# jacobkrantz/IVLN-CE

Measured on AMD Instinct MI355X. Metric: env-steps/sec (batched MapCMA fwd+bwd) at 1/2/4/8 MI355X; t-nDTW parity, higher is better.
Workload: dtype f32

## Files before the change

### include/ivln_hip.h

```cpp
#ifndef IVLN_HIP_H
#define IVLN_HIP_H
#include <stdint.h>
#ifdef __cplusplus
extern "C" {
#endif

#define IVLN_OK 0
#define IVLN_E_INVALID -1
#define IVLN_E_HIP -2
#define IVLN_E_KEYSPACE -3
#define IVLN_E_CAPACITY -4
#define IVLN_E_UNSUPPORTED -5

const char* ivln_strerror(int code);
int ivln_version(void);

typedef struct ivln_mapper ivln_mapper;

int ivln_mapper_create(int B_max, int H, int W, double vfov_rad, double height_m, double width_m,
                       double res_m, int64_t world_capacity, int64_t table_cells, ivln_mapper** out);
int ivln_mapper_destroy(ivln_mapper* m);
int ivln_mapper_reset(ivln_mapper* m, void* stream);

int ivln_mapper_set_launch_width(ivln_mapper* m, int local_blocks, int world_blocks);
// ... 65 lines not shown
    int64_t ws_floats;
    int defer_epilogue;
    int* splits_used;
    int tile_override;
    const float* A_packed;
    int no_xcd_remap;
    int grp_imgs;
    int64_t a_grp_stride, a_packed_grp_stride;
    int no_wide_epilogue;
    float* stat_partials;
    int* stat_tiles;
    const void* A_split;
    int64_t a_split_grp_stride;
    int split_ok;
    const int32_t* img_run_flags;
    const void* fuse_A_split;
    int64_t fuse_a_grp_stride;
    const float* fuse_scale;
    const float* fuse_shift;
    int fuse_M;
    int residual_after_relu;
    int real_taps;
    int pool2;
    const uint8_t* map_sem_u8;
} ivln_gemm_desc;

int ivln_gemm_f32(const ivln_gemm_desc* desc, void* stream);
int64_t ivln_conv_split_words(int M, int Cin, int KS);
int ivln_conv_split_weights_f32(const float* W, int M, int Cin, int KS, void* out, void* stream);
int64_t ivln_conv_stem_split_words(int M, int Cin);
int ivln_conv_stem_split_weights_f32(const float* W, int M, int Cin, void* out, void* stream);
int ivln_conv_split_counters(double* flops, long long* launches, int reset);
int ivln_conv_split_kinds(long long* out4, int reset);

int ivln_family_timing_begin(int max_launches);
int ivln_family_timing_end(double* total_ms, int* launches, int* dropped);
int ivln_family_timing_report(char* buf, int cap);
const char* ivln_family_kernel_names(void);
int64_t ivln_conv_packed_floats(int M, int Cin, int KS);
int ivln_conv_pack_weights_f32(const float* W, int M, int Cin, int KS, float* out, void* stream);

typedef struct ivln_gn_conv_desc {
    const float* x;
    int splits;
    int64_t slab_stride;
    const float* gamma;
    const float* beta;
    const float* x2;
    int splits2;
    int64_t slab_stride2;
    const float* gamma2;
    const float* beta2;
    const float* residual;
    int N, C, H, W, groups;
    float eps;
    int relu;
    int pool;
    float* act_out;
    const float* wa;
    int Cout_a, ka, stride_a, pad_a;
    float* ya;
    const float* wb;
    int Cout_b, stride_b;
    float* yb;
    const float* x0;
    int splits0;
// ... 292 lines not shown
```

### ivln-ce_amd/csrc/conv_bf3.hip

```cpp
#include <stdlib.h>

#include <type_traits>

#include "gemm_common.h"
#include "residency.h"

namespace {

typedef __bf16 bf16x8 __attribute__((ext_vector_type(8)));
typedef int v4i __attribute__((ext_vector_type(4)));
typedef int v2i __attribute__((ext_vector_type(2)));

constexpr int PIXB = 112;
constexpr int CB = 16;

__host__ __device__ constexpr int bf3_taps_padded(int KS) { return KS == 7 ? 54 : (KS == 3 ? 9 : (KS == 2 ? 4 : 1)); }
__host__ __device__ constexpr int bf3_gx0(int KS) { return KS == 2 ? 0 : 4; }
__host__ __device__ constexpr int bf3_xoff(int KS) { return KS == 2 ? 0 : 4 - KS / 2; }
__host__ __device__ constexpr int bf3_stage_chunks(int KS) { return KS == 1 ? 4 : 1; }

__device__ __forceinline__ uint32_t bf16_rne_bits(float v, bool& fin) {
    const uint32_t u = __float_as_uint(v);
    fin = (u & 0x7F800000u) != 0x7F800000u;
    uint32_t hb = (u + 0x7FFFu + ((u >> 16) & 1u)) & 0xFFFF0000u;
// ... 1067 lines not shown
    if (!attr_done) {
        if (hipFuncSetAttribute((const void*)kern, hipFuncAttributeMaxDynamicSharedMemorySize, (int)lds) != hipSuccess) return IVLN_E_HIP;
        attr_done = true;
    }
    const int tiles_w = d.Wout / 8, tiles_h = d.Hout / 4;
    dim3 grid(tiles_w * tiles_h * nimg, (d.M + 31) / 32, 1);
    IVLN_LAUNCH_FAMILY_NAMED("k_conv7_pool_bf3", kern, grid, dim3(64 * NW), lds, s, d, (const unsigned char*)d.A_split, tiles_w, tiles_h, nimg);
    return IVLN_OK;
}

int bf3_conv7_pool_launch(ivln_gemm_desc& d, hipStream_t s) {
    if (d.bmode != BMODE_CONV_K7 || d.amode != AMODE_MK || d.dmode != DMODE_NCHW || d.dil != 1 || d.stride != 1 || d.pad != 3 ||
        d.Hout != d.Hin || d.Wout != d.Win || d.K != d.Cin * 49 || d.HoWo != d.Hout * d.Wout || d.N % d.HoWo != 0)
        return IVLN_E_UNSUPPORTED;
    if ((d.Hout & 3) || (d.Wout & 7) || !d.scale || !d.shift || !d.relu || d.residual || d.accumulate || d.residual_after_relu || d.defer_epilogue ||
        d.splits > 1 || d.stat_partials || d.img_run_flags || d.fuse_A_split || d.grp_imgs > 0 || d.Cin > 8 * CB)
        return IVLN_E_UNSUPPORTED;
    const int nimg = d.N / d.HoWo;
    const int64_t tiles = (int64_t)nimg * (d.Hout / 4) * (d.Wout / 8);
    if (tiles >= (int64_t)1 << 30) return IVLN_E_UNSUPPORTED;
    d.splits = 1;
    if (d.map_sem_u8) {
        if (d.Cin != 14 || (int64_t)nimg * d.HoWo >= (int64_t)1 << 31) return IVLN_E_UNSUPPORTED;
        return launch_conv7_pool<1, true>(d, s, nimg);
    }
    if ((d.in_img_stride & 3) || (((uintptr_t)d.B) & 15) || (int64_t)nimg * d.in_img_stride * 4 >= (int64_t)1 << 31) return IVLN_E_UNSUPPORTED;
    const int nch = (d.Cin + CB - 1) / CB;
    if (nch == 1) return launch_conv7_pool<1, false>(d, s, nimg);
    if (nch == 2) return launch_conv7_pool<2, false>(d, s, nimg);
    if (nch <= 4) return launch_conv7_pool<4, false>(d, s, nimg);
    return launch_conv7_pool<8, false>(d, s, nimg);
}

template <bool WT>
__global__ __launch_bounds__(WT ? 256 : 512, 2) void k_conv1x1_bf3_ks(const ivln_gemm_desc p, const unsigned char* a_split, long long a_grp_bytes) {
    constexpr int NW = WT ? 4 : 8, TN = 4, DA = 4, BN = 128;
    constexpr int LDT = BN + 4;
    constexpr unsigned OOB = 0x80000000u;
    extern __shared__ __attribute__((aligned(16))) unsigned char smem[];
    const int t = threadIdx.x, lane = t & 63;
    const int wave = __builtin_amdgcn_readfirstlane(t >> 6);
    const int half = lane >> 5, l31 = lane & 31;
    const BlockId bid = xcd_block_id(p.no_xcd_remap);
    const int n0 = WT ? (bid.y * NW + wave) * BN : bid.y * BN, m0 = bid.x * 32;
    const int nch = p.Cin / CB;
    const int HW = p.HoWo;
    const int cpw = WT ? nch : (nch + NW - 1) / NW;
    const int c0 = WT ? 0 : min(nch, wave * cpw), c1 = WT ? nch : min(nch, c0 + cpw);
    const int n_img0 = min(n0, p.N - 1) / HW;
    const int grp = p.grp_imgs > 0 ? n_img0 / p.grp_imgs : 0;

    const int nq = n0 + 4 * l31;
    const int qimg = nq / HW, qpp = nq - qimg * HW;
    const unsigned hw4 = (unsigned)HW * 4u;
    const unsigned xvo = nq < p.N ? (unsigned)(((int64_t)qimg * p.in_img_stride + qpp + (int64_t)(8 * half) * HW) * 4) : OOB;
    const __amdgpu_buffer_rsrc_t rB = bf3_rsrc(p.B);
    auto load_x = [&](int c, v4i (&xb)[8]) {
        const int so = c * CB * HW * 4;
#pragma unroll
        for (int j = 0; j < 8; ++j) xb[j] = __builtin_amdgcn_raw_buffer_load_b128(rB, (int)xvo, so + j * (int)hw4, 0);
    };
    const int mt = min(m0 / 32, (p.M + 31) / 32 - 1);
    const __amdgpu_buffer_rsrc_t rA = bf3_rsrc(a_split + (int64_t)grp * a_grp_bytes + (int64_t)mt * nch * (3 * 1024));
    const int c_last = max(c1 - 1, 0);
    auto load_a = [&](int c, v4i (&ab)[3]) {
#pragma unroll
        for (int pl = 0; pl < 3; ++pl) ab[pl] = __builtin_amdgcn_raw_buffer_load_b128(rA, (min(c, c_last) * 3 + pl) * 1024 + lane * 16, 0, 0);
    };
    f32x16 acc[TN];
#pragma unroll
    for (int tn = 0; tn < TN; ++tn)
#pragma unroll
        for (int i = 0; i < 16; ++i) acc[tn][i] = 0.f;

#ifdef BF3_TIMING
    const unsigned long long ts0 = lane == 0 ? wall_clock64() : 0ull;
    unsigned long long ts1 = ts0, tc_split = 0, tc_load = 0, tc_mfma = 0;
#endif
    if (c0 < c1 && (!WT || n0 < p.N)) {
        v4i xb[2][8], ab[DA][3];
#pragma unroll
        for (int d = 0; d < DA; ++d) load_a(c0 + d, ab[d]);
        load_x(c0, xb[0]);
        load_x(min(c0 + 1, c_last), xb[1]);
#ifdef BF3_TIMING
        __builtin_amdgcn_s_waitcnt(0);
        ts1 = lane == 0 ? wall_clock64() : 0ull;
#endif
        for (int cc = c0; cc < c1; cc += DA) {
#pragma unroll
            for (int k = 0; k < DA; ++k) {
                const int c = cc + k;
                v4i bq[TN][3];
                bf16x8 a[3];
#ifdef BF3_TIMING
                const unsigned long long tl0 = __builtin_readcyclecounter();
#endif
                if (c < c1) {
#pragma unroll
                    for (int e = 0; e < 4; ++e)
#pragma unroll
                        for (int i = 0; i < 4; ++i) {
                            uint32_t H, M, L;
#ifdef BF3_PROBE_NO_SPLIT
                            H = xb[k & 1][2 * i][e], M = xb[k & 1][2 * i + 1][e], L = H ^ M;
#else
                            split3_pair(__int_as_float(xb[k & 1][2 * i][e]), __int_as_float(xb[k & 1][2 * i + 1][e]), H, M, L);
#endif
                            bq[e][0][i] = (int)H, bq[e][1][i] = (int)M, bq[e][2][i] = (int)L;
                        }
#pragma unroll
                    for (int pl = 0; pl < 3; ++pl) a[pl] = __builtin_bit_cast(bf16x8, ab[k][pl]);
                }
                __builtin_amdgcn_sched_barrier(0);
#ifdef BF3_TIMING
                const unsigned long long tl1 = __builtin_readcyclecounter();
                __builtin_amdgcn_sched_barrier(0);
#endif
                load_x(min(c + 2, c_last), xb[k & 1]);
                load_a(c + DA, ab[k]);
                __builtin_amdgcn_sched_barrier(0);
#ifdef BF3_TIMING
                const unsigned long long tl2 = __builtin_readcyclecounter();
                __builtin_amdgcn_sched_barrier(0);
#endif
                if (c < c1) {
#define IVLN_BF3_PROD(PA, PB)                            \
    _Pragma("unroll") for (int tn = 0; tn < TN; ++tn)    \
        acc[tn] = __builtin_amdgcn_mfma_f32_32x32x16_bf16(a[PA], __builtin_bit_cast(bf16x8, bq[tn][PB]), acc[tn], 0, 0, 0)
#ifdef BF3_PROBE_NO_MFMA
                    IVLN_BF3_PROD(0, 0);
#else
                    IVLN_BF3_PROD(0, 2);
                    IVLN_BF3_PROD(1, 1);
                    IVLN_BF3_PROD(2, 0);
                    IVLN_BF3_PROD(0, 1);
                    IVLN_BF3_PROD(1, 0);
                    IVLN_BF3_PROD(0, 0);
#endif
#undef IVLN_BF3_PROD
                }
#ifdef BF3_TIMING
                __builtin_amdgcn_sched_barrier(0);
                const unsigned long long tl3 = __builtin_readcyclecounter();
                tc_split += tl1 - tl0, tc_load += tl2 - tl1, tc_mfma += tl3 - tl2;
#endif
            }
        }
    }
#ifdef BF3_TIMING
    const unsigned long long ts2 = lane == 0 ? wall_clock64() : 0ull;
#endif
    const bool up = p.dmode == DMODE_NCHW_UP2X4;
    if (WT && up) {
        const int n = n0 + 4 * l31;
        if (n < p.N) {
            const int img = n / HW, pp = n - img * HW;
            const int ho = pp / p.Wout, wo = pp - ho * p.Wout;
#pragma unroll
            for (int r = 0; r < 16; r += 2) {
                const int m = m0 + 4 * half + (r & 3) + 8 * (r >> 2);
                if (m >= p.M) continue;
                const int co = m >> 2, a = (m >> 1) & 1;
                const int64_t addr = (((int64_t)img * p.Ctot + co) * (2 * p.Hout) + 2 * ho + a) * (2 * p.Wout) + 2 * wo;
                float v[8];
#pragma unroll
                for (int e = 0; e < 4; ++e) v[2 * e] = acc[e][r], v[2 * e + 1] = acc[e][r + 1];
                const float sc = p.scale ? p.scale[co] : 1.f, sh = p.shift ? p.shift[co] : 0.f;
#pragma unroll
                for (int e = 0; e < 8; ++e) v[e] = p.scale ? fmaf(v[e], sc, sh) : v[e] + sh;
                if (p.residual) {
                    const float4 r0 = *reinterpret_cast<const float4*>(p.residual + addr), r1 = *reinterpret_cast<const float4*>(p.residual + addr + 4);
                    v[0] += r0.x, v[1] += r0.y, v[2] += r0.z, v[3] += r0.w, v[4] += r1.x, v[5] += r1.y, v[6] += r1.z, v[7] += r1.w;
                }
                if (p.relu) {
#pragma unroll
                    for (int e = 0; e < 8; ++e) v[e] = fmaxf(v[e], 0.f);
                }
                *reinterpret_cast<float4*>(p.D + addr) = make_float4(v[0], v[1], v[2], v[3]);
                *reinterpret_cast<float4*>(p.D + addr + 4) = make_float4(v[4], v[5], v[6], v[7]);
            }
        }
    } else
    if constexpr (WT) {
        const int n = n0 + 4 * l31;
        const int img = min(n, p.N - 1) / HW, pp = n - img * HW;
        const int mrem = n < p.N ? p.M - m0 - 4 * half : 0;
        const int me0 = (p.grp_imgs > 0 ? (img / p.grp_imgs) * p.M : 0) + m0 + 4 * half;
        const unsigned off0 = (unsigned)(((img * p.Ctot + m0 + 4 * half) * HW + pp) * 4);
        const __amdgpu_buffer_rsrc_t rR = bf3_rsrc(p.residual), rS = bf3_rsrc(p.scale), rH = bf3_rsrc(p.shift), rD = bf3_rsrc(p.D);
        const bool has_res = p.residual != nullptr, has_sc = p.scale != nullptr, has_sh = p.shift != nullptr;
        const float relu_lo = p.relu ? 0.f : -__builtin_huge_valf();
        const bool res_post = p.residual_after_relu != 0;
        v4i rres[16];
        float esc[16], esh[16];
#pragma unroll
        for (int r = 0; r < 16; ++r) {
            const int cs = (r & 3) + 8 * (r >> 2);
            const bool ok = cs < mrem;
            esc[r] = __int_as_float(__builtin_amdgcn_raw_buffer_load_b32(rS, ok && has_sc ? me0 * 4 : (int)OOB, cs * 4, 0));
            esh[r] = __int_as_float(__builtin_amdgcn_raw_buffer_load_b32(rH, ok && has_sh ? me0 * 4 : (int)OOB, cs * 4, 0));
            rres[r] = __builtin_amdgcn_raw_buffer_load_b128(rR, ok && has_res ? (int)off0 : (int)OOB, cs * HW * 4, 0);
        }
#pragma unroll
        for (int r = 0; r < 16; ++r) {
            const int cs = (r & 3) + 8 * (r >> 2);
            float4 v = make_float4(acc[0][r], acc[1][r], acc[2][r], acc[3][r]);
            const float sc = has_sc ? esc[r] : 1.f, sh = esh[r];
            v.x = fmaf(v.x, sc, sh), v.y = fmaf(v.y, sc, sh), v.z = fmaf(v.z, sc, sh), v.w = fmaf(v.w, sc, sh);
            const float r0 = __int_as_float(rres[r][0]), r1 = __int_as_float(rres[r][1]), r2 = __int_as_float(rres[r][2]), r3 = __int_as_float(rres[r][3]);
            v.x += res_post ? 0.f : r0, v.y += res_post ? 0.f : r1, v.z += res_post ? 0.f : r2, v.w += res_post ? 0.f : r3;
            const float lo = relu_lo;
            v.x = fmaxf(v.x, lo), v.y = fmaxf(v.y, lo), v.z = fmaxf(v.z, lo), v.w = fmaxf(v.w, lo);
            v.x += res_post ? r0 : 0.f, v.y += res_post ? r1 : 0.f, v.z += res_post ? r2 : 0.f, v.w += res_post ? r3 : 0.f;
            v4i o;
            o[0] = __float_as_int(v.x), o[1] = __float_as_int(v.y), o[2] = __float_as_int(v.z), o[3] = __float_as_int(v.w);
            __builtin_amdgcn_raw_buffer_store_b128(o, rD, cs < mrem ? (int)off0 : (int)OOB, cs * HW * 4, 0);
            BF3_STORE_GUARD();
        }
    } else if (up) {
        float* const red = reinterpret_cast<float*>(smem);
#pragma unroll
        for (int tn = 0; tn < TN; ++tn)
#pragma unroll
            for (int r = 0; r < 16; ++r)
                red[(wave * 32 + (r & 3) + 8 * (r >> 2) + 4 * half) * LDT + tn * 32 + l31] = acc[tn][r];
        __syncthreads();
#pragma unroll
        for (int it = 0; it < 2; ++it) {
            const int item = t + it * 512, r = item >> 6, j = item & 63;
            const int ml = 2 * r, nl = 2 * j, n = n0 + nl;
            const int e0 = nl & 3, q = nl >> 2;
            float4 v = make_float4(0.f, 0.f, 0.f, 0.f);
#pragma unroll
            for (int w = 0; w < NW; ++w) {
                const float* r0 = red + (w * 32 + ml) * LDT + q;
                const float* r1 = r0 + LDT;
                v.x += r0[e0 * 32], v.y += r1[e0 * 32], v.z += r0[(e0 + 1) * 32], v.w += r1[(e0 + 1) * 32];
            }
            if (m0 + ml < p.M && n < p.N) {
                const int img = n / HW, pp = n - img * HW;
                const int ho = pp / p.Wout, wo = pp - ho * p.Wout;
                const int co = (m0 + ml) >> 2, a = r & 1;
                const int64_t addr = (((int64_t)img * p.Ctot + co) * (2 * p.Hout) + 2 * ho + a) * (2 * p.Wout) + 2 * wo;
                if (p.scale) {
                    const float sc = p.scale[co], sh = p.shift[co];
                    v.x = fmaf(v.x, sc, sh), v.y = fmaf(v.y, sc, sh), v.z = fmaf(v.z, sc, sh), v.w = fmaf(v.w, sc, sh);
                } else if (p.shift) {
                    const float sh = p.shift[co];
                    v.x += sh, v.y += sh, v.z += sh, v.w += sh;
                }
                if (p.residual) {
                    const float4 rr = *reinterpret_cast<const float4*>(p.residual + addr);
                    v.x += rr.x, v.y += rr.y, v.z += rr.z, v.w += rr.w;
                }
                if (p.relu) v.x = fmaxf(v.x, 0.f), v.y = fmaxf(v.y, 0.f), v.z = fmaxf(v.z, 0.f), v.w = fmaxf(v.w, 0.f);
                *reinterpret_cast<float4*>(p.D + addr) = v;
            }
        }
    } else {
    constexpr int ITEMS = 2;
    v4i rres[ITEMS];
    float esc[ITEMS], esh[ITEMS];
    int eoff[ITEMS];
    const __amdgpu_buffer_rsrc_t rR = bf3_rsrc(p.residual), rS = bf3_rsrc(p.scale), rH = bf3_rsrc(p.shift);
    const bool has_res = p.residual != nullptr, has_sc = p.scale != nullptr, has_sh = p.shift != nullptr;
    auto request = [&](int it) {
        const int item = t + it * 512, ml = item >> 5, q = item & 31;
        const int m = m0 + ml, n = n0 + 4 * q;
        const bool ok = m < p.M && n < p.N;
        const int img = n / HW, pp = n - img * HW;
        const int off = (img * p.Ctot + m) * HW + pp;
        const int me = p.grp_imgs > 0 ? (img / p.grp_imgs) * p.M + m : m;
        eoff[it] = ok ? off : -1;
        esc[it] = __int_as_float(__builtin_amdgcn_raw_buffer_load_b32(rS, ok && has_sc ? me * 4 : (int)OOB, 0, 0));
        esh[it] = __int_as_float(__builtin_amdgcn_raw_buffer_load_b32(rH, ok && has_sh ? me * 4 : (int)OOB, 0, 0));
        rres[it] = __builtin_amdgcn_raw_buffer_load_b128(rR, ok && has_res ? off * 4 : (int)OOB, 0, 0);
    };
#pragma unroll
    for (int it = 0; it < ITEMS; ++it) request(it);
    float* const red = reinterpret_cast<float*>(smem);
#pragma unroll
    for (int tn = 0; tn < TN; ++tn)
#pragma unroll
        for (int r = 0; r < 16; ++r)
            red[(wave * 32 + (r & 3) + 8 * (r >> 2) + 4 * half) * LDT + tn * 32 + l31] = acc[tn][r];
    __syncthreads();
#pragma unroll
    for (int it = 0; it < ITEMS; ++it) {
        const int item = t + it * 512, ml = item >> 5, q = item & 31;
        float4 v = make_float4(0.f, 0.f, 0.f, 0.f);
#pragma unroll
        for (int w = 0; w < NW; ++w) {
            const float* rr = red + (w * 32 + ml) * LDT + q;
            v.x += rr[0], v.y += rr[32], v.z += rr[64], v.w += rr[96];
        }
        if (eoff[it] >= 0) {
            const int64_t addr = eoff[it];
            const float sc = esc[it], sh = esh[it];
            if (p.scale) v.x = fmaf(v.x, sc, sh), v.y = fmaf(v.y, sc, sh), v.z = fmaf(v.z, sc, sh), v.w = fmaf(v.w, sc, sh);
            else if (p.shift) v.x += sh, v.y += sh, v.z += sh, v.w += sh;
            const bool res_pre = p.residual && !p.residual_after_relu, res_post = p.residual && p.residual_after_relu;
            if (res_pre)
                v.x += __int_as_float(rres[it][0]), v.y += __int_as_float(rres[it][1]), v.z += __int_as_float(rres[it][2]),
                    v.w += __int_as_float(rres[it][3]);
            if (p.accumulate) {
                const float4 ra = *reinterpret_cast<const float4*>(p.D + addr);
                v.x += ra.x, v.y += ra.y, v.z += ra.z, v.w += ra.w;
            }
            if (p.relu) v.x = fmaxf(v.x, 0.f), v.y = fmaxf(v.y, 0.f), v.z = fmaxf(v.z, 0.f), v.w = fmaxf(v.w, 0.f);
            if (res_post)
                v.x += __int_as_float(rres[it][0]), v.y += __int_as_float(rres[it][1]), v.z += __int_as_float(rres[it][2]),
                    v.w += __int_as_float(rres[it][3]);
            *reinterpret_cast<float4*>(p.D + addr) = v;
        }
    }
    }
#ifdef BF3_TIMING
    if (lane == 0) {
        __builtin_amdgcn_s_waitcnt(0);
        const unsigned long long ts3 = wall_clock64();
        const int b = ((blockIdx.y * gridDim.x + blockIdx.x) * NW + wave) & 8191;
        g_bf3_stamp[b * 8 + 0] = ts1 - ts0;
        g_bf3_stamp[b * 8 + 1] = ts2 - ts1;
        g_bf3_stamp[b * 8 + 2] = ts3 - ts2;
        g_bf3_stamp[b * 8 + 3] = ts0;
        g_bf3_stamp[b * 8 + 4] = tc_split;
        g_bf3_stamp[b * 8 + 5] = tc_load;
        g_bf3_stamp[b * 8 + 6] = tc_mfma;
    }
#endif
}

int bf3_1x1_ks_launch(ivln_gemm_desc& d, hipStream_t s, int mode, int form_pin = -1) {
    if (d.stride != 1 || d.pad != 0 || d.Cin % CB != 0 || d.Cin < 4 * CB || d.stat_partials || d.splits > 1) return IVLN_E_UNSUPPORTED;
    if ((d.HoWo & 3) || (d.in_img_stride & 3) || ((((uintptr_t)d.B) | ((uintptr_t)d.D) | ((uintptr_t)d.residual)) & 15)) return IVLN_E_UNSUPPORTED;
    const int64_t nimg = d.N / d.HoWo;
    if (nimg * d.in_img_stride * 4 >= (int64_t)1 << 31 || nimg * d.Ctot * d.HoWo * 4 >= (int64_t)1 << 31) return IVLN_E_UNSUPPORTED;
    if (d.grp_imgs > 0 && ((int64_t)d.grp_imgs * d.HoWo) % 128 != 0) return IVLN_E_UNSUPPORTED;
    const int nch = d.Cin / CB;
    constexpr const char* form_env = nullptr;
    bool wt = nch <= 16;
    constexpr int maxwg0 = 2;
    if (nch == 32 && (int64_t)((d.N + 127) / 128) * ((d.M + 31) / 32) > maxwg0 * (int64_t)ivln_cu_count()) wt = true;
    if (form_env) wt = form_env[0] == 'w';
    if (form_pin >= 0) wt = form_pin == 1;
    if (wt && nch > 64) wt = false;
    if (wt && d.accumulate) return IVLN_E_UNSUPPORTED;
    const int64_t mtiles = (d.M + 31) / 32;
    const int64_t wgs = wt ? (int64_t)((d.N + 511) / 512) * mtiles : (int64_t)((d.N + 127) / 128) * mtiles;
    constexpr int maxwg_env = 2;
    if ((d.N + 127) / 128 > 65535) return IVLN_E_UNSUPPORTED;
    if (mode == 0) {
        if (!wt && (d.Cin < 32 * CB || wgs > maxwg_env * (int64_t)ivln_cu_count() || wgs < ivln_cu_count() / 2)) return IVLN_E_UNSUPPORTED;
        if (wt && wgs < ivln_cu_count()) return IVLN_E_UNSUPPORTED;
    }
    d.splits = 1;
    const unsigned char* a = (const unsigned char*)d.A_split;
    const long long gb = (long long)(d.a_split_grp_stride * 4);
    if (wt) {
        constexpr size_t lds = 0;
        dim3 grid((unsigned)mtiles, (unsigned)((d.N + 511) / 512), 1);
        IVLN_LAUNCH_FAMILY(k_conv1x1_bf3_ks<true>, grid, dim3(256), lds, s, d, a, gb);
    } else {
        constexpr size_t lds = (size_t)8 * 32 * (128 + 4) * 4;
        static bool attr_done = false;
        if (!attr_done) {
            if (hipFuncSetAttribute((const void*)k_conv1x1_bf3_ks<false>, hipFuncAttributeMaxDynamicSharedMemorySize, (int)lds) != hipSuccess) return IVLN_E_HIP;
            attr_done = true;
        }
        dim3 grid((unsigned)mtiles, (unsigned)((d.N + 127) / 128), 1);
        IVLN_LAUNCH_FAMILY(k_conv1x1_bf3_ks<false>, grid, dim3(512), lds, s, d, a, gb);
    }
    return IVLN_OK;
}

__global__ __launch_bounds__(256) void k_conv_bf3_pack(const float* __restrict__ W, int M, int Cin, int KS, uint16_t* __restrict__ out,
                                                       int64_t total) {
    const int64_t idx = (int64_t)blockIdx.x * 256 + threadIdx.x;
    if (idx >= total) return;
    const int KK = KS * KS, KKP = bf3_taps_padded(KS), nch = (Cin + CB - 1) / CB;
    const int e = (int)(idx & 7), lane = (int)((idx >> 3) & 63);
    int64_t q = idx >> 9;
    const int pl = (int)(q % 3);
    q /= 3;
    const int r = (int)(q % KKP);
    q /= KKP;
    const int c = (int)(q % nch);
    const int mt = (int)(q / nch);
    const int m = mt * 32 + (lane & 31), ci = c * CB + (lane >> 5) * 8 + e;
    const float v = (m < M && ci < Cin && r < KK) ? W[((int64_t)m * Cin + ci) * KK + r] : 0.f;
    uint32_t h, mm, l;
    split3(v, h, mm, l);
    out[idx] = (uint16_t)(pl == 0 ? h : (pl == 1 ? mm : l));
}

template <int KS, int TM, int WM, int WN, int PTH, int PTW, int IMGS, int DA, int ST = 1>
int launch_bf3(const ivln_gemm_desc& d, hipStream_t s, const unsigned char* a_split, int64_t grp_bytes, int nimg, int cps) {
    constexpr int NTB = 64 * WM * WN, BM = 32 * TM * WM, BN = 64 * WN;
    constexpr int PH = ST == 2 ? PTH + 1 : PTH + KS - 1, PWR = ST == 2 ? PTW + 1 : PTW + KS - 1;
    constexpr int NPIX = IMGS * (ST == 2 ? 4 : 1) * PH * PWR * bf3_stage_chunks(KS);
    constexpr size_t lds = (size_t)(NPIX * PIXB > 32 * (BN + 4) * 4 ? NPIX * PIXB : 32 * (BN + 4) * 4);
    if constexpr (lds > 160 * 1024) {
        return IVLN_E_UNSUPPORTED;
    } else {
    auto kern = k_conv_bf3<KS, TM, WM, WN, PTH, PTW, IMGS, DA, false, ST>;
    static bool attr_done = false;
// ... 574 lines not shown
extern "C" int ivln_conv_bf3_stamps(unsigned long long* host, int n) {
    if (hipMemcpyFromSymbol(host, HIP_SYMBOL(g_bf3_stamp), sizeof(unsigned long long) * n) != hipSuccess) return -1;
    void* dp = nullptr;
    if (hipGetSymbolAddress(&dp, HIP_SYMBOL(g_bf3_stamp)) != hipSuccess) return -1;
    return hipMemset(dp, 0, sizeof(g_bf3_stamp)) == hipSuccess ? 0 : -1;
}
#endif

int ivln_conv_bf3_launch(ivln_gemm_desc& d, hipStream_t s, bool force) {
    constexpr bool disabled = false;
    if (!d.A_split || (disabled && !force)) return IVLN_E_UNSUPPORTED;
    if (d.pool2) {
        const int rc = bf3_conv7_pool_launch(d, s);
        if (rc == IVLN_OK) g_bf3_flops += 2.0 * d.M * (double)d.N * d.K, ++g_bf3_launches, ++g_bf3_kind[1];
        return rc;
    }
    const int KS = d.bmode == BMODE_CONV1X1 ? 1 : conv_ks(d.bmode);
    if ((KS != 1 && KS != 2 && KS != 3 && KS != 7) || d.amode != AMODE_MK || d.dil != 1) return IVLN_E_UNSUPPORTED;
    if (KS == 7 && d.stride == 2) {
        const int rc = bf3_stem_launch(d, s);
        if (rc == IVLN_OK) g_bf3_flops += 2.0 * d.M * (double)d.N * d.K, ++g_bf3_launches, ++g_bf3_kind[0];
        if (rc == IVLN_OK && d.stat_tiles) *d.stat_tiles = 0;
        return rc;
    }
    const bool up1 = KS == 1 && d.dmode == DMODE_NCHW_UP2X4;
    if (!up1 && d.dmode != (KS == 2 ? DMODE_NCHW_UP2X4 : DMODE_NCHW)) return IVLN_E_UNSUPPORTED;
    if (up1) {
        static const bool convt_off1 = getenv("IVLN_BF3_CONVT") && getenv("IVLN_BF3_CONVT")[0] == '0';
        if ((convt_off1 && !force) || (d.M & 3) || d.Ctot * 4 != d.M || d.grp_imgs > 0 || d.accumulate || d.residual_after_relu || d.defer_epilogue ||
            d.splits > 1 || d.stat_partials || d.img_run_flags || d.fuse_A_split || (d.Wout & 3) || d.stride != 1 || d.pad != 0 || d.Hout != d.Hin ||
            d.Wout != d.Win || d.K != d.Cin || d.HoWo != d.Hout * d.Wout || d.N % d.HoWo != 0)
            return IVLN_E_UNSUPPORTED;
        const int ovu = d.tile_override;
        const int rc = bf3_1x1_ks_launch(d, s, (force || ovu == 11 || ovu == 12 || ovu == 13) ? 1 : 0, ovu == 12 ? 0 : (ovu == 13 ? 1 : -1));
        if (rc == IVLN_OK) g_bf3_flops += 2.0 * d.M * (double)d.N * d.K, ++g_bf3_launches, ++g_bf3_kind[d.Cin / CB <= 16 ? 3 : 2];
        return rc;
    }
    const double flops_of = 2.0 * d.M * (double)d.N * d.K * (KS == 2 && d.real_taps > 0 ? d.real_taps / 16.0 : 1.0);
    if (KS == 2) {
        if (d.stride != 1 || d.pad != 0 || d.Hout != d.Hin || d.Wout != d.Win || (d.M & 3) || d.grp_imgs > 0 || d.stat_partials || d.defer_epilogue ||
            d.splits > 1 || d.fuse_A_split || d.residual_after_relu || d.img_run_flags || d.K != d.Cin * 4 || d.HoWo != d.Hout * d.Wout ||
            d.N % d.HoWo != 0 || (d.Wout & 3) || d.Wout < 8 || (((uintptr_t)d.D | (uintptr_t)d.residual) & 15) || d.Ctot * 4 != d.M)
            return IVLN_E_UNSUPPORTED;
        const int nimg2 = d.N / d.HoWo;
        if ((int64_t)nimg2 * d.in_img_stride >= (int64_t)1 << 31) return IVLN_E_UNSUPPORTED;
        static const bool convt_off = getenv("IVLN_BF3_CONVT") && getenv("IVLN_BF3_CONVT")[0] == '0';
        if (convt_off && !force) return IVLN_E_UNSUPPORTED;
        const int ov2 = d.tile_override;
        if (ov2 < 20) {
            const int rc = bf3_ks_launch(d, s, nimg2, (ov2 == 10 || ov2 == 15) ? 1 : 0);
            if (rc != IVLN_E_UNSUPPORTED || ov2 == 10 || ov2 == 15) {
                if (rc == IVLN_OK) g_bf3_flops += flops_of, ++g_bf3_launches, ++g_bf3_kind[1];
                return rc;
            }
        }
        const int CUS2 = ivln_cu_count();
        auto blocks2 = [&](int cfg) {
            const Bf3Px t = bf3_px(kBf3BN[cfg], d.Wout);
            return (int64_t)((d.Wout + t.ptw - 1) / t.ptw) * ((d.Hout + t.pth - 1) / t.pth) * ((nimg2 + t.imgs - 1) / t.imgs) *
                   ((d.M + kBf3BM[cfg] - 1) / kBf3BM[cfg]);
        };
        int cfg2 = blocks2(3) >= CUS2 ? 3 : (blocks2(2) >= CUS2 ? 2 : (blocks2(5) >= CUS2 ? 5 : 4));
        if (ov2 >= 20 && ov2 < 20 + kBf3Cfgs) cfg2 = ov2 - 20;
        if (!force && blocks2(cfg2) < CUS2 / 2) return IVLN_E_UNSUPPORTED;
        d.splits = 1;
        const int rc = launch_bf3_ks<2>(d, s, (const unsigned char*)d.A_split, d.a_split_grp_stride * 4, nimg2, cfg2, (d.Cin + CB - 1) / CB);
        if (rc == IVLN_OK) g_bf3_flops += flops_of, ++g_bf3_launches, ++g_bf3_kind[0];
        return rc;
    }
    static const int ks1_env = getenv("IVLN_BF3_1X1_KS") ? atoi(getenv("IVLN_BF3_1X1_KS")) : -1;
    const int ov = d.tile_override;
    const bool post = d.residual_after_relu != 0;
    const bool ins1 = ov == 11 || ov == 12 || ov == 13 || post, ins3 = ov == 10 || ov == 14 || ov == 15;
    if (KS == 1 && ov < 20 && (ks1_env != 0 || ins1) && d.splits <= 1 && !d.defer_epilogue && d.HoWo == d.Hout * d.Wout &&
        d.K == d.Cin && d.N % d.HoWo == 0 && d.Hout == d.Hin && d.Wout == d.Win) {
        const int rc = bf3_1x1_ks_launch(d, s, (ks1_env == 1 || ins1) ? 1 : 0, ov == 12 ? 0 : (ov == 13 ? 1 : -1));
        if (rc != IVLN_E_UNSUPPORTED || ins1) {
            if (rc == IVLN_OK) g_bf3_flops += 2.0 * d.M * (double)d.N * d.K, ++g_bf3_launches, ++g_bf3_kind[ov == 13 ? 3 : (ov == 12 ? 2 : (d.Cin / CB <= 16 ? 3 : 2))];
            if (rc == IVLN_OK && d.stat_tiles) *d.stat_tiles = 0;
            return rc;
        }
    }
    if (ins1 || (ins3 && KS != 3)) return IVLN_E_UNSUPPORTED;
    if (KS == 1) {
        if ((d.stride != 1 && d.stride != 2) || d.pad != 0 || d.Hout != (d.Hin - 1) / d.stride + 1 || d.Wout != (d.Win - 1) / d.stride + 1 || d.M < 64)
            return IVLN_E_UNSUPPORTED;
    } else if (KS == 3 && d.stride == 2) {
        static const bool s2_off = getenv("IVLN_BF3_S2") && getenv("IVLN_BF3_S2")[0] == '0';
        if ((s2_off && !force) || d.pad != 1 || d.Hin != 2 * d.Hout || d.Win != 2 * d.Wout || d.Cin % CB != 0 || d.fuse_A_split || d.stat_partials ||
            d.img_run_flags)
            return IVLN_E_UNSUPPORTED;
    } else if (d.stride != 1 || d.pad != KS / 2 || d.Hout != d.Hin || d.Wout != d.Win) {
        return IVLN_E_UNSUPPORTED;
    }
    const bool s2 = KS == 3 && d.stride == 2;
    if (d.K != d.Cin * KS * KS || d.HoWo != d.Hout * d.Wout || d.N % d.HoWo != 0) return IVLN_E_UNSUPPORTED;
    if (d.defer_epilogue || d.splits > 1 || (d.Wout & 3) || d.Wout < 8 || (((uintptr_t)d.D | (uintptr_t)d.residual | (uintptr_t)d.ws) & 15))
        return IVLN_E_UNSUPPORTED;
    const int nimg = d.N / d.HoWo;
    if ((int64_t)nimg * d.in_img_stride >= (int64_t)1 << 31) return IVLN_E_UNSUPPORTED;
    if (d.fuse_A_split) {
        static const bool fuse_off = getenv("IVLN_BF3_FUSE") && getenv("IVLN_BF3_FUSE")[0] == '0';
        if (fuse_off || KS != 3 || (d.M != 64 && d.M != 128) || d.Cin % CB != 0 || d.Wout % 32 != 0 || d.Hout % 4 != 0 || d.fuse_M <= 0 ||
            d.fuse_M % 32 != 0 || d.stat_partials || d.accumulate || !d.relu || d.img_run_flags)
            return IVLN_E_UNSUPPORTED;
        if ((int64_t)nimg * d.Ctot * d.HoWo * 4 >= (int64_t)1 << 31 || (d.grp_imgs > 0 && nimg % d.grp_imgs != 0)) return IVLN_E_UNSUPPORTED;
        d.splits = 1;
        const unsigned char* a = (const unsigned char*)d.A_split;
        const int64_t gb = d.a_split_grp_stride * 4;
        constexpr int px_env = 0;
        const int64_t wg128 = (int64_t)nimg * (d.Wout / 32) * (d.Hout / 4);
// ... 133 lines not shown
```

Measured before the change: 2461.

## Template 1x1 split-bf16 conv kernel on pixel tile width and pick it adaptively

Measured after the change: 2470, median of 6. No clear change (+0.4%).

```diff
diff --git a/include/ivln_hip.h b/include/ivln_hip.h
--- a/include/ivln_hip.h
+++ b/include/ivln_hip.h
@@ -121,6 +121,7 @@
 int ivln_conv_stem_split_weights_f32(const float* W, int M, int Cin, void* out, void* stream);
 int ivln_conv_split_counters(double* flops, long long* launches, int reset);
 int ivln_conv_split_kinds(long long* out4, int reset);
+int ivln_conv1x1_split_tile(int M, long long N, int Cin, int* wave_tiles, int* tn);
 
 int ivln_family_timing_begin(int max_launches);
 int ivln_family_timing_end(double* total_ms, int* launches, int* dropped);
diff --git a/ivln-ce_amd/csrc/conv_bf3.hip b/ivln-ce_amd/csrc/conv_bf3.hip
--- a/ivln-ce_amd/csrc/conv_bf3.hip
+++ b/ivln-ce_amd/csrc/conv_bf3.hip
@@ -1123,9 +1123,35 @@
     return launch_conv7_pool<8, false>(d, s, nimg);
 }
 
-template <bool WT>
+template <int TN> struct bf3_words;
+template <> struct bf3_words<4> {
+    typedef v4i vec;
+    static __device__ __forceinline__ vec load(__amdgpu_buffer_rsrc_t r, int vo, int so) { return __builtin_amdgcn_raw_buffer_load_b128(r, vo, so, 0); }
+    static __device__ __forceinline__ void store(vec v, __amdgpu_buffer_rsrc_t r, int vo, int so) { __builtin_amdgcn_raw_buffer_store_b128(v, r, vo, so, 0); }
+    static __device__ __forceinline__ int get(const vec& v, int e) { return v[e]; }
+    static __device__ __forceinline__ void set(vec& v, int e, int x) { v[e] = x; }
+};
+template <> struct bf3_words<2> {
+    typedef v2i vec;
+    static __device__ __forceinline__ vec load(__amdgpu_buffer_rsrc_t r, int vo, int so) { return __builtin_amdgcn_raw_buffer_load_b64(r, vo, so, 0); }
+    static __device__ __forceinline__ void store(vec v, __amdgpu_buffer_rsrc_t r, int vo, int so) { __builtin_amdgcn_raw_buffer_store_b64(v, r, vo, so, 0); }
+    static __device__ __forceinline__ int get(const vec& v, int e) { return v[e]; }
+    static __device__ __forceinline__ void set(vec& v, int e, int x) { v[e] = x; }
+};
+template <> struct bf3_words<1> {
+    typedef int vec;
+    static __device__ __forceinline__ vec load(__amdgpu_buffer_rsrc_t r, int vo, int so) { return __builtin_amdgcn_raw_buffer_load_b32(r, vo, so, 0); }
+    static __device__ __forceinline__ void store(vec v, __amdgpu_buffer_rsrc_t r, int vo, int so) { __builtin_amdgcn_raw_buffer_store_b32(v, r, vo, so, 0); }
+    static __device__ __forceinline__ int get(const vec& v, int) { return v; }
+    static __device__ __forceinline__ void set(vec& v, int, int x) { v = x; }
+};
+
+template <bool WT, int TN>
 __global__ __launch_bounds__(WT ? 256 : 512, 2) void k_conv1x1_bf3_ks(const ivln_gemm_desc p, const unsigned char* a_split, long long a_grp_bytes) {
-    constexpr int NW = WT ? 4 : 8, TN = 4, DA = 4, BN = 128;
+    static_assert(TN == 4 || TN == 2 || TN == 1, "pixel tiles per wave");
+    typedef bf3_words<TN> PX;
+    typedef typename PX::vec xvec;
+    constexpr int NW = WT ? 4 : 8, DA = 4, BN = 32 * TN;
     constexpr int LDT = BN + 4;
     constexpr unsigned OOB = 0x80000000u;
     extern __shared__ __attribute__((aligned(16))) unsigned char smem[];
@@ -1141,15 +1167,15 @@
     const int n_img0 = min(n0, p.N - 1) / HW;
     const int grp = p.grp_imgs > 0 ? n_img0 / p.grp_imgs : 0;
 
-    const int nq = n0 + 4 * l31;
+    const int nq = n0 + TN * l31;
     const int qimg = nq / HW, qpp = nq - qimg * HW;
     const unsigned hw4 = (unsigned)HW * 4u;
     const unsigned xvo = nq < p.N ? (unsigned)(((int64_t)qimg * p.in_img_stride + qpp + (int64_t)(8 * half) * HW) * 4) : OOB;
     const __amdgpu_buffer_rsrc_t rB = bf3_rsrc(p.B);
-    auto load_x = [&](int c, v4i (&xb)[8]) {
+    auto load_x = [&](int c, xvec (&xb)[8]) {
         const int so = c * CB * HW * 4;
 #pragma unroll
-        for (int j = 0; j < 8; ++j) xb[j] = __builtin_amdgcn_raw_buffer_load_b128(rB, (int)xvo, so + j * (int)hw4, 0);
+        for (int j = 0; j < 8; ++j) xb[j] = PX::load(rB, (int)xvo, so + j * (int)hw4);
     };
     const int mt = min(m0 / 32, (p.M + 31) / 32 - 1);
     const __amdgpu_buffer_rsrc_t rA = bf3_rsrc(a_split + (int64_t)grp * a_grp_bytes + (int64_t)mt * nch * (3 * 1024));
@@ -1169,7 +1195,8 @@
     unsigned long long ts1 = ts0, tc_split = 0, tc_load = 0, tc_mfma = 0;
 #endif
     if (c0 < c1 && (!WT || n0 < p.N)) {
-        v4i xb[2][8], ab[DA][3];
+        xvec xb[2][8];
+        v4i ab[DA][3];
 #pragma unroll
         for (int d = 0; d < DA; ++d) load_a(c0 + d, ab[d]);
         load_x(c0, xb[0]);
@@ -1189,14 +1216,14 @@
 #endif
                 if (c < c1) {
 #pragma unroll
-                    for (int e = 0; e < 4; ++e)
+                    for (int e = 0; e < TN; ++e)
 #pragma unroll
                         for (int i = 0; i < 4; ++i) {
                             uint32_t H, M, L;
 #ifdef BF3_PROBE_NO_SPLIT
-                            H = xb[k & 1][2 * i][e], M = xb[k & 1][2 * i + 1][e], L = H ^ M;
+                            H = PX::get(xb[k & 1][2 * i], e), M = PX::get(xb[k & 1][2 * i + 1], e), L = H ^ M;
 #else
-                            split3_pair(__int_as_float(xb[k & 1][2 * i][e]), __int_as_float(xb[k & 1][2 * i + 1][e]), H, M, L);
+                            split3_pair(__int_as_float(PX::get(xb[k & 1][2 * i], e)), __int_as_float(PX::get(xb[k & 1][2 * i + 1], e)), H, M, L);
 #endif
                             bq[e][0][i] = (int)H, bq[e][1][i] = (int)M, bq[e][2][i] = (int)L;
                         }
@@ -1244,7 +1271,7 @@
 #endif
     const bool up = p.dmode == DMODE_NCHW_UP2X4;
     if (WT && up) {
-        const int n = n0 + 4 * l31;
+        const int n = n0 + TN * l31;
         if (n < p.N) {
             const int img = n / HW, pp = n - img * HW;
             const int ho = pp / p.Wout, wo = pp - ho * p.Wout;
@@ -1254,27 +1281,40 @@
                 if (m >= p.M) continue;
                 const int co = m >> 2, a = (m >> 1) & 1;
                 const int64_t addr = (((int64_t)img * p.Ctot + co) * (2 * p.Hout) + 2 * ho + a) * (2 * p.Wout) + 2 * wo;
-                float v[8];
-#pragma unroll
-                for (int e = 0; e < 4; ++e) v[2 * e] = acc[e][r], v[2 * e + 1] = acc[e][r + 1];
+                float v[2 * TN];
+#pragma unroll
+                for (int e = 0; e < TN; ++e) v[2 * e] = acc[e][r], v[2 * e + 1] = acc[e][r + 1];
                 const float sc = p.scale ? p.scale[co] : 1.f, sh = p.shift ? p.shift[co] : 0.f;
 #pragma unroll
-                for (int e = 0; e < 8; ++e) v[e] = p.scale ? fmaf(v[e], sc, sh) : v[e] + sh;
+                for (int e = 0; e < 2 * TN; ++e) v[e] = p.scale ? fmaf(v[e], sc, sh) : v[e] + sh;
                 if (p.residual) {
-                    const float4 r0 = *reinterpret_cast<const float4*>(p.residual + addr), r1 = *reinterpret_cast<const float4*>(p.residual + addr + 4);
-                    v[0] += r0.x, v[1] += r0.y, v[2] += r0.z, v[3] += r0.w, v[4] += r1.x, v[5] += r1.y, v[6] += r1.z, v[7] += r1.w;
+                    if constexpr (TN == 1) {
+                        const float2 r0 = *reinterpret_cast<const float2*>(p.residual + addr);
+                        v[0] += r0.x, v[1] += r0.y;
+                    } else {
+#pragma unroll
+                        for (int h = 0; h < TN / 2; ++h) {
+                            const float4 r0 = *reinterpret_cast<const float4*>(p.residual + addr + 4 * h);
+                            v[4 * h] += r0.x, v[4 * h + 1] += r0.y, v[4 * h + 2] += r0.z, v[4 * h + 3] += r0.w;
+                        }
+                    }
                 }
                 if (p.relu) {
 #pragma unroll
-                    for (int e = 0; e < 8; ++e) v[e] = fmaxf(v[e], 0.f);
-                }
-                *reinterpret_cast<float4*>(p.D + addr) = make_float4(v[0], v[1], v[2], v[3]);
-                *reinterpret_cast<float4*>(p.D + addr + 4) = make_float4(v[4], v[5], v[6], v[7]);
+                    for (int e = 0; e < 2 * TN; ++e) v[e] = fmaxf(v[e], 0.f);
+                }
+                if constexpr (TN == 1) {
+                    *reinterpret_cast<float2*>(p.D + addr) = make_float2(v[0], v[1]);
+                } else {
+#pragma unroll
+                    for (int h = 0; h < TN / 2; ++h)
+                        *reinterpret_cast<float4*>(p.D + addr + 4 * h) = make_float4(v[4 * h], v[4 * h + 1], v[4 * h + 2], v[4 * h + 3]);
+                }
             }
         }
     } else
     if constexpr (WT) {
-        const int n = n0 + 4 * l31;
+        const int n = n0 + TN * l31;
         const int img = min(n, p.N - 1) / HW, pp = n - img * HW;
         const int mrem = n < p.N ? p.M - m0 - 4 * half : 0;
         const int me0 = (p.grp_imgs > 0 ? (img / p.grp_imgs) * p.M : 0) + m0 + 4 * half;
@@ -1283,7 +1323,7 @@
         const bool has_res = p.residual != nullptr, has_sc = p.scale != nullptr, has_sh = p.shift != nullptr;
         const float relu_lo = p.relu ? 0.f : -__builtin_huge_valf();
         const bool res_post = p.residual_after_relu != 0;
-        v4i rres[16];
+        xvec rres[16];
         float esc[16], esh[16];
 #pragma unroll
         for (int r = 0; r < 16; ++r) {
@@ -1291,22 +1331,24 @@
             const bool ok = cs < mrem;
             esc[r] = __int_as_float(__builtin_amdgcn_raw_buffer_load_b32(rS, ok && has_sc ? me0 * 4 : (int)OOB, cs * 4, 0));
             esh[r] = __int_as_float(__builtin_amdgcn_raw_buffer_load_b32(rH, ok && has_sh ? me0 * 4 : (int)OOB, cs * 4, 0));
-            rres[r] = __builtin_amdgcn_raw_buffer_load_b128(rR, ok && has_res ? (int)off0 : (int)OOB, cs * HW * 4, 0);
+            rres[r] = PX::load(rR, ok && has_res ? (int)off0 : (int)OOB, cs * HW * 4);
         }
 #pragma unroll
         for (int r = 0; r < 16; ++r) {
             const int cs = (r & 3) + 8 * (r >> 2);
-            float4 v = make_float4(acc[0][r], acc[1][r], acc[2][r], acc[3][r]);
             const float sc = has_sc ? esc[r] : 1.f, sh = esh[r];
-            v.x = fmaf(v.x, sc, sh), v.y = fmaf(v.y, sc, sh), v.z = fmaf(v.z, sc, sh), v.w = fmaf(v.w, sc, sh);
-            const float r0 = __int_as_float(rres[r][0]), r1 = __int_as_float(rres[r][1]), r2 = __int_as_float(rres[r][2]), r3 = __int_as_float(rres[r][3]);
-            v.x += res_post ? 0.f : r0, v.y += res_post ? 0.f : r1, v.z += res_post ? 0.f : r2, v.w += res_post ? 0.f : r3;
             const float lo = relu_lo;
-            v.x = fmaxf(v.x, lo), v.y = fmaxf(v.y, lo), v.z = fmaxf(v.z, lo), v.w = fmaxf(v.w, lo);
-            v.x += res_post ? r0 : 0.f, v.y += res_post ? r1 : 0.f, v.z += res_post ? r2 : 0.f, v.w += res_post ? r3 : 0.f;
-            v4i o;
-            o[0] = __float_as_int(v.x), o[1] = __float_as_int(v.y), o[2] = __float_as_int(v.z), o[3] = __float_as_int(v.w);
-            __builtin_amdgcn_raw_buffer_store_b128(o, rD, cs < mrem ? (int)off0 : (int)OOB, cs * HW * 4, 0);
+            xvec o;
+#pragma unroll
+            for (int e = 0; e < TN; ++e) {
+                float v = fmaf(acc[e][r], sc, sh);
+                const float re = __int_as_float(PX::get(rres[r], e));
+                v += res_post ? 0.f : re;
+                v = fmaxf(v, lo);
+                v += res_post ? re : 0.f;
+                PX::set(o, e, __float_as_int(v));
+            }
+            PX::store(o, rD, cs < mrem ? (int)off0 : (int)OOB, cs * HW * 4);
             BF3_STORE_GUARD();
         }
     } else if (up) {
@@ -1317,17 +1359,19 @@
             for (int r = 0; r < 16; ++r)
                 red[(wave * 32 + (r & 3) + 8 * (r >> 2) + 4 * half) * LDT + tn * 32 + l31] = acc[tn][r];
         __syncthreads();
-#pragma unroll
-        for (int it = 0; it < 2; ++it) {
-            const int item = t + it * 512, r = item >> 6, j = item & 63;
+        constexpr int PAIRS = BN / 2, NITEM = 16 * PAIRS;
+#pragma unroll
+        for (int it = 0; it < (NITEM + 511) / 512; ++it) {
+            const int item = t + it * 512, r = item / PAIRS, j = item % PAIRS;
+            if (NITEM < 512 && item >= NITEM) break;
             const int ml = 2 * r, nl = 2 * j, n = n0 + nl;
-            const int e0 = nl & 3, q = nl >> 2;
+            const int i0 = (nl % TN) * 32 + nl / TN, i1 = ((nl + 1) % TN) * 32 + (nl + 1) / TN;
             float4 v = make_float4(0.f, 0.f, 0.f, 0.f);
 #pragma unroll
             for (int w = 0; w < NW; ++w) {
-                const float* r0 = red + (w * 32 + ml) * LDT + q;
+                const float* r0 = red + (w * 32 + ml) * LDT;
                 const float* r1 = r0 + LDT;
-                v.x += r0[e0 * 32], v.y += r1[e0 * 32], v.z += r0[(e0 + 1) * 32], v.w += r1[(e0 + 1) * 32];
+                v.x += r0[i0], v.y += r1[i0], v.z += r0[i1], v.w += r1[i1];
             }
             if (m0 + ml < p.M && n < p.N) {
                 const int img = n / HW, pp = n - img * HW;
@@ -1350,16 +1394,17 @@
             }
         }
     } else {
-    constexpr int ITEMS = 2;
+    constexpr int QN = BN / 4, NITEM = 32 * QN;
+    constexpr int ITEMS = (NITEM + 511) / 512;
     v4i rres[ITEMS];
     float esc[ITEMS], esh[ITEMS];
     int eoff[ITEMS];
     const __amdgpu_buffer_rsrc_t rR = bf3_rsrc(p.residual), rS = bf3_rsrc(p.scale), rH = bf3_rsrc(p.shift);
     const bool has_res = p.residual != nullptr, has_sc = p.scale != nullptr, has_sh = p.shift != nullptr;
     auto request = [&](int it) {
-        const int item = t + it * 512, ml = item >> 5, q = item & 31;
+        const int item = t + it * 512, ml = item / QN, q = item % QN;
         const int m = m0 + ml, n = n0 + 4 * q;
-        const bool ok = m < p.M && n < p.N;
+        const bool ok = item < NITEM && m < p.M && n < p.N;
         const int img = n / HW, pp = n - img * HW;
         const int off = (img * p.Ctot + m) * HW + pp;
         const int me = p.grp_imgs > 0 ? (img / p.grp_imgs) * p.M + m : m;
@@ -1379,12 +1424,13 @@
     __syncthreads();
 #pragma unroll
     for (int it = 0; it < ITEMS; ++it) {
-        const int item = t + it * 512, ml = item >> 5, q = item & 31;
+        const int item = t + it * 512, ml = (item / QN) & 31, q = item % QN;
+        auto col = [](int px) { return (px % TN) * 32 + px / TN; };
         float4 v = make_float4(0.f, 0.f, 0.f, 0.f);
 #pragma unroll
         for (int w = 0; w < NW; ++w) {
-            const float* rr = red + (w * 32 + ml) * LDT + q;
-            v.x += rr[0], v.y += rr[32], v.z += rr[64], v.w += rr[96];
+            const float* rr = red + (w * 32 + ml) * LDT;
+            v.x += rr[col(4 * q)], v.y += rr[col(4 * q + 1)], v.z += rr[col(4 * q + 2)], v.w += rr[col(4 * q + 3)];
         }
         if (eoff[it] >= 0) {
             const int64_t addr = eoff[it];
@@ -1423,47 +1469,86 @@
 #endif
 }
 
-int bf3_1x1_ks_launch(ivln_gemm_desc& d, hipStream_t s, int mode, int form_pin = -1) {
+static int g_bf3_1x1_last[2] = {0, 4};
+
+static inline bool bf3_1x1_tile_pin(int ov) { return ov >= 30 && ov <= 35; }
+static inline int bf3_1x1_form_pin(int ov) { return ov == 12 ? 0 : (ov == 13 ? 1 : (bf3_1x1_tile_pin(ov) ? (ov - 30) / 3 : -1)); }
+static inline int bf3_1x1_tn_pin(int ov) { return bf3_1x1_tile_pin(ov) ? 4 >> ((ov - 30) % 3) : 0; }
+
+struct Bf3Tile1x1 {
+    bool wt;
+    int tn;
+};
+static int bf3_1x1_ks_choose(int M, int64_t N, int Cin, int mode, int form_pin, int tn_pin, Bf3Tile1x1* out) {
+    const int nch = Cin / CB;
+    const int64_t mtiles = (M + 31) / 32, CUS = ivln_cu_count();
+    bool wt = nch <= 16;
+    constexpr int maxwg0 = 2;
+    if (nch == 32 && ((N + 127) / 128) * mtiles > maxwg0 * CUS) wt = true;
+    if (form_pin >= 0) wt = form_pin == 1;
+    if (wt && nch > 64) wt = false;
+    auto wgs = [&](int tn) { return ((N + (wt ? 4 : 1) * 32 * tn - 1) / ((wt ? 4 : 1) * 32 * tn)) * mtiles; };
+    constexpr int maxwg_env = 2;
+    if (mode == 0) {
+        if (!wt && (Cin < 32 * CB || wgs(4) > maxwg_env * CUS || wgs(1) < CUS)) return IVLN_E_UNSUPPORTED;
+        if (wt && wgs(4) < CUS) return IVLN_E_UNSUPPORTED;
+    }
+    const int64_t need = CUS;
+    int tn = wgs(4) >= need ? 4 : (wgs(2) >= need ? 2 : (wgs(1) >= need ? 1 : 4));
+    if (tn_pin) tn = tn_pin;
+    out->wt = wt, out->tn = tn;
+    return IVLN_OK;
+}
+
+extern "C" int ivln_conv1x1_split_tile(int M, long long N, int Cin, int* wave_tiles, int* tn) {
+    if (M <= 0 || N <= 0 || Cin % CB != 0 || Cin < 4 * CB) return IVLN_E_UNSUPPORTED;
+    Bf3Tile1x1 c;
+    const int rc = bf3_1x1_ks_choose(M, N, Cin, 0, -1, 0, &c);
+    if (rc != IVLN_OK) return rc;
+    if (wave_tiles) *wave_tiles = c.wt ? 1 : 0;
+    if (tn) *tn = c.tn;
+    return IVLN_OK;
+}
+
+template <bool WT, int TN>
+int launch_1x1_ks(const ivln_gemm_desc& d, hipStream_t s) {
+    constexpr int NWT = WT ? 4 : 1;
+    constexpr size_t lds = WT ? 0 : (size_t)8 * 32 * (32 * TN + 4) * 4;
+    auto kern = k_conv1x1_bf3_ks<WT, TN>;
+    if (lds > 48 * 1024) {
+        static bool attr_done = false;
+        if (!attr_done) {
+            if (hipFuncSetAttribute((const void*)kern, hipFuncAttributeMaxDynamicSharedMemorySize, (int)lds) != hipSuccess) return IVLN_E_HIP;
+            attr_done = true;
+        }
+    }
+    const int64_t ptiles = ((int64_t)d.N + NWT * 32 * TN - 1) / (NWT * 32 * TN);
+    if (ptiles > 65535) return IVLN_E_UNSUPPORTED;
+    dim3 grid((unsigned)((d.M + 31) / 32), (unsigned)ptiles, 1);
+    const unsigned char* a = (const unsigned char*)d.A_split;
+    const long long gb = (long long)(d.a_split_grp_stride * 4);
+    IVLN_LAUNCH_FAMILY_NAMED("k_conv1x1_bf3_ks", kern, grid, dim3(WT ? 256 : 512), lds, s, d, a, gb);
+    return IVLN_OK;
+}
+
+int bf3_1x1_ks_launch(ivln_gemm_desc& d, hipStream_t s, int mode, int form_pin = -1, int tn_pin = 0) {
     if (d.stride != 1 || d.pad != 0 || d.Cin % CB != 0 || d.Cin < 4 * CB || d.stat_partials || d.splits > 1) return IVLN_E_UNSUPPORTED;
     if ((d.HoWo & 3) || (d.in_img_stride & 3) || ((((uintptr_t)d.B) | ((uintptr_t)d.D) | ((uintptr_t)d.residual)) & 15)) return IVLN_E_UNSUPPORTED;
     const int64_t nimg = d.N / d.HoWo;
     if (nimg * d.in_img_stride * 4 >= (int64_t)1 << 31 || nimg * d.Ctot * d.HoWo * 4 >= (int64_t)1 << 31) return IVLN_E_UNSUPPORTED;
-    if (d.grp_imgs > 0 && ((int64_t)d.grp_imgs * d.HoWo) % 128 != 0) return IVLN_E_UNSUPPORTED;
-    const int nch = d.Cin / CB;
-    constexpr const char* form_env = nullptr;
-    bool wt = nch <= 16;
-    constexpr int maxwg0 = 2;
-    if (nch == 32 && (int64_t)((d.N + 127) / 128) * ((d.M + 31) / 32) > maxwg0 * (int64_t)ivln_cu_count()) wt = true;
-    if (form_env) wt = form_env[0] == 'w';
-    if (form_pin >= 0) wt = form_pin == 1;
-    if (wt && nch > 64) wt = false;
-    if (wt && d.accumulate) return IVLN_E_UNSUPPORTED;
-    const int64_t mtiles = (d.M + 31) / 32;
-    const int64_t wgs = wt ? (int64_t)((d.N + 511) / 512) * mtiles : (int64_t)((d.N + 127) / 128) * mtiles;
-    constexpr int maxwg_env = 2;
-    if ((d.N + 127) / 128 > 65535) return IVLN_E_UNSUPPORTED;
-    if (mode == 0) {
-        if (!wt && (d.Cin < 32 * CB || wgs > maxwg_env * (int64_t)ivln_cu_count() || wgs < ivln_cu_count() / 2)) return IVLN_E_UNSUPPORTED;
-        if (wt && wgs < ivln_cu_count()) return IVLN_E_UNSUPPORTED;
+    Bf3Tile1x1 c;
+    const int rc = bf3_1x1_ks_choose(d.M, d.N, d.Cin, mode, form_pin, tn_pin, &c);
+    if (rc != IVLN_OK) return rc;
+    if (c.wt && d.accumulate) return IVLN_E_UNSUPPORTED;
+    if (d.grp_imgs > 0) {
+        const int64_t gpx = (int64_t)d.grp_imgs * d.HoWo;
+        while (!tn_pin && c.tn > 1 && gpx % (32 * c.tn) != 0) c.tn >>= 1;
+        if (gpx % (32 * c.tn) != 0) return IVLN_E_UNSUPPORTED;
     }
     d.splits = 1;
-    const unsigned char* a = (const unsigned char*)d.A_split;
-    const long long gb = (long long)(d.a_split_grp_stride * 4);
-    if (wt) {
-        constexpr size_t lds = 0;
-        dim3 grid((unsigned)mtiles, (unsigned)((d.N + 511) / 512), 1);
-        IVLN_LAUNCH_FAMILY(k_conv1x1_bf3_ks<true>, grid, dim3(256), lds, s, d, a, gb);
-    } else {
-        constexpr size_t lds = (size_t)8 * 32 * (128 + 4) * 4;
-        static bool attr_done = false;
-        if (!attr_done) {
-            if (hipFuncSetAttribute((const void*)k_conv1x1_bf3_ks<false>, hipFuncAttributeMaxDynamicSharedMemorySize, (int)lds) != hipSuccess) return IVLN_E_HIP;
-            attr_done = true;
-        }
-        dim3 grid((unsigned)mtiles, (unsigned)((d.N + 127) / 128), 1);
-        IVLN_LAUNCH_FAMILY(k_conv1x1_bf3_ks<false>, grid, dim3(512), lds, s, d, a, gb);
-    }
-    return IVLN_OK;
+    g_bf3_1x1_last[0] = c.wt ? 1 : 0, g_bf3_1x1_last[1] = c.tn;
+    if (c.wt) return c.tn == 4 ? launch_1x1_ks<true, 4>(d, s) : (c.tn == 2 ? launch_1x1_ks<true, 2>(d, s) : launch_1x1_ks<true, 1>(d, s));
+    return c.tn == 4 ? launch_1x1_ks<false, 4>(d, s) : (c.tn == 2 ? launch_1x1_ks<false, 2>(d, s) : launch_1x1_ks<false, 1>(d, s));
 }
 
 __global__ __launch_bounds__(256) void k_conv_bf3_pack(const float* __restrict__ W, int M, int Cin, int KS, uint16_t* __restrict__ out,
@@ -2104,8 +2189,9 @@
             d.Wout != d.Win || d.K != d.Cin || d.HoWo != d.Hout * d.Wout || d.N % d.HoWo != 0)
             return IVLN_E_UNSUPPORTED;
         const int ovu = d.tile_override;
-        const int rc = bf3_1x1_ks_launch(d, s, (force || ovu == 11 || ovu == 12 || ovu == 13) ? 1 : 0, ovu == 12 ? 0 : (ovu == 13 ? 1 : -1));
-        if (rc == IVLN_OK) g_bf3_flops += 2.0 * d.M * (double)d.N * d.K, ++g_bf3_launches, ++g_bf3_kind[d.Cin / CB <= 16 ? 3 : 2];
+        const int rc = bf3_1x1_ks_launch(d, s, (force || ovu == 11 || ovu == 12 || ovu == 13 || bf3_1x1_tile_pin(ovu)) ? 1 : 0, bf3_1x1_form_pin(ovu),
+                                         bf3_1x1_tn_pin(ovu));
+        if (rc == IVLN_OK) g_bf3_flops += 2.0 * d.M * (double)d.N * d.K, ++g_bf3_launches, ++g_bf3_kind[g_bf3_1x1_last[0] ? 3 : 2];
         return rc;
     }
     const double flops_of = 2.0 * d.M * (double)d.N * d.K * (KS == 2 && d.real_taps > 0 ? d.real_taps / 16.0 : 1.0);
@@ -2143,12 +2229,12 @@
     static const int ks1_env = getenv("IVLN_BF3_1X1_KS") ? atoi(getenv("IVLN_BF3_1X1_KS")) : -1;
     const int ov = d.tile_override;
     const bool post = d.residual_after_relu != 0;
-    const bool ins1 = ov == 11 || ov == 12 || ov == 13 || post, ins3 = ov == 10 || ov == 14 || ov == 15;
-    if (KS == 1 && ov < 20 && (ks1_env != 0 || ins1) && d.splits <= 1 && !d.defer_epilogue && d.HoWo == d.Hout * d.Wout &&
+    const bool ins1 = ov == 11 || ov == 12 || ov == 13 || bf3_1x1_tile_pin(ov) || post, ins3 = ov == 10 || ov == 14 || ov == 15;
+    if (KS == 1 && (ov < 20 || bf3_1x1_tile_pin(ov)) && (ks1_env != 0 || ins1) && d.splits <= 1 && !d.defer_epilogue && d.HoWo == d.Hout * d.Wout &&
         d.K == d.Cin && d.N % d.HoWo == 0 && d.Hout == d.Hin && d.Wout == d.Win) {
-        const int rc = bf3_1x1_ks_launch(d, s, (ks1_env == 1 || ins1) ? 1 : 0, ov == 12 ? 0 : (ov == 13 ? 1 : -1));
+        const int rc = bf3_1x1_ks_launch(d, s, (ks1_env == 1 || ins1) ? 1 : 0, bf3_1x1_form_pin(ov), bf3_1x1_tn_pin(ov));
         if (rc != IVLN_E_UNSUPPORTED || ins1) {
-            if (rc == IVLN_OK) g_bf3_flops += 2.0 * d.M * (double)d.N * d.K, ++g_bf3_launches, ++g_bf3_kind[ov == 13 ? 3 : (ov == 12 ? 2 : (d.Cin / CB <= 16 ? 3 : 2))];
+            if (rc == IVLN_OK) g_bf3_flops += 2.0 * d.M * (double)d.N * d.K, ++g_bf3_launches, ++g_bf3_kind[g_bf3_1x1_last[0] ? 3 : 2];
             if (rc == IVLN_OK && d.stat_tiles) *d.stat_tiles = 0;
             return rc;
         }
```
